# mchitten/keto

Measured on AMD Instinct MI355X. Metric: permission checks/sec (batched, whole node) + traversal HBM GB/s vs roofline, higher is better.
Workload: dtype u32 ids / u64 bitmasks (integer)

## Files before the change

include/ketogpu.h:

```cpp
#ifndef KETOGPU_H
#define KETOGPU_H

#include <stddef.h>
#include <stdint.h>

#ifdef __cplusplus
extern "C" {
#endif

#define KETOGPU_ABI_VERSION 9

#define KETOGPU_OK 0
#define KETOGPU_ENOTFOUND 1
#define KETOGPU_EINVAL 2
#define KETOGPU_EDEVICE 3
#define KETOGPU_ENOMEM 4
#define KETOGPU_ECOLLISION 5

#define KETOGPU_SUBJECT_ID 0
#define KETOGPU_SUBJECT_SET 1
#define KETOGPU_SUBJECT_NIL (-1)

#define KETOGPU_NODE_NONE 0xFFFFFFFFu
#define KETOGPU_NODE_NOT_OWNED 0xFFFFFFFEu
// ... 197 lines not shown
int ketogpu_host_alloc(size_t bytes, void **out);
void ketogpu_host_free(void *p);

typedef struct ketogpu_multi ketogpu_multi;
int ketogpu_multi_new(const ketogpu_snapshot *s, const int32_t *devices, size_t num_devices,
                      const ketogpu_engine_opts *opts, ketogpu_multi **out);
void ketogpu_multi_free(ketogpu_multi *m);
size_t ketogpu_multi_size(const ketogpu_multi *m);
ketogpu_engine *ketogpu_multi_engine(ketogpu_multi *m, size_t i);
int ketogpu_multi_check_ids(ketogpu_multi *m, const uint32_t *roots, const uint32_t *targets, size_t n,
                            uint64_t *allowed_bits, uint64_t *flagged_bits);
int ketogpu_multi_check_ids_packed24(ketogpu_multi *m, const void *packed, size_t n, uint64_t *allowed_bits,
                                     uint64_t *flagged_bits);
void ketogpu_multi_range(size_t n, size_t parts, size_t i, size_t *begin, size_t *end);

int ketogpu_queries_upload(ketogpu_engine *e, const uint32_t *roots, const uint32_t *targets,
                           size_t n, ketogpu_queries **out);
int ketogpu_queries_run(ketogpu_engine *e, ketogpu_queries *q);
int ketogpu_queries_download(ketogpu_engine *e, const ketogpu_queries *q, uint64_t *allowed_bits,
                             uint64_t *flagged_bits);
int ketogpu_queries_run_async(ketogpu_engine *e, ketogpu_queries *q, int *queued);
int ketogpu_engine_wait(ketogpu_engine *e);
int ketogpu_engine_piped_full_requests(ketogpu_engine *e, uint64_t *out);
void ketogpu_queries_free(ketogpu_queries *q);

typedef struct {
    uint64_t checks;
    uint64_t rounds;
    uint64_t levels;
    uint64_t frontier_entries;
    uint64_t interior_edges;
    uint64_t rev_edges;
    uint64_t touched;
    uint64_t bytes_push;
    uint64_t bytes_pull;
    uint64_t bytes_total;
    double ms_push;
    double ms_pull;
    double ms_total;
    uint64_t push_launches;
    uint64_t overflow_retries;
    uint64_t spilled_units;
    uint64_t unit_rows;
    uint64_t unit_edges;
    uint64_t unit_rev;
    uint64_t bytes_unit;
// ... 255 lines not shown
} ketogpu_tier_steps;
int ketogpu_tier_new_steps(const ketogpu_tier_steps *steps, ketogpu_comm *comm, const ketogpu_tier_opts *opts,
                           ketogpu_tier **out);

int ketogpu_expand(const ketogpu_snapshot *s, const ketogpu_subject *subject, int32_t rest_depth,
                   ketogpu_tree **out);

#define KETOGPU_NODE_UNION 0
#define KETOGPU_NODE_LEAF 1
typedef struct {
    int32_t type;
    uint32_t num_children;
    ketogpu_subject subject;
} ketogpu_tree_node;
int ketogpu_tree_nodes(const ketogpu_tree *t, const ketogpu_tree_node **nodes, size_t *n);
int ketogpu_tree_json(const ketogpu_tree *t, char **json);
void ketogpu_tree_free(ketogpu_tree *t);

const char *ketogpu_last_error(void);
int ketogpu_abi_version(void);
void ketogpu_free(void *p);
int ketogpu_device_count(void);
int ketogpu_probe_random_lines(int device, uint64_t table_bytes, uint64_t requests, int reps, double *ms_per_launch);

#ifdef __cplusplus
}
#endif
#endif
```

keto_amd/_lib.py:

```python
import ctypes as C
import os

HERE = os.path.dirname(os.path.abspath(__file__))
LIB_PATH = os.environ.get("KETOGPU_LIB") or os.path.join(HERE, "libketogpu.so")

OK, ENOTFOUND, EINVAL, EDEVICE, ENOMEM, ECOLLISION = 0, 1, 2, 3, 4, 5
SUBJECT_ID, SUBJECT_SET, SUBJECT_NIL = 0, 1, -1
NODE_NONE = 0xFFFFFFFF
NODE_NOT_OWNED = 0xFFFFFFFE
BUILD_SORT = 1
ORDER_NULLS_LAST = 2
ORDERS = {"sqlite": 0, "mysql-bin": 0, "cockroach": 0, "postgres": ORDER_NULLS_LAST}
BUILD_WRITABLE = 4
WRITE_REASONS = {0: "applied", 1: "not_writable", 2: "wildcard", 3: "poison", 4: "class", 5: "ambiguous",
                 6: "full", 7: "reserve", 8: "fanout"}
NODE_UNION, NODE_LEAF = 0, 1


class KetoError(Exception):

    NAMES = {ENOTFOUND: "not_found", EINVAL: "invalid", EDEVICE: "device", ENOMEM: "nomem", ECOLLISION: "collision"}

    def __init__(self, code, msg=""):
        super().__init__(f"{self.NAMES.get(code, code)}: {msg}")
# ... 286 lines not shown
    "ketogpu_snapshot_set_namespaces": (C.c_int, [vp, C.POINTER(Namespace), sz, C.POINTER(vp)]),
    "ketogpu_snapshot_write": (C.c_int, [vp, C.POINTER(RowBatch), C.POINTER(RowBatch), C.POINTER(WriteResult)]),
    "ketogpu_snapshot_version": (C.c_uint64, [vp]),
    "ketogpu_engine_sync": (C.c_int, [vp, C.POINTER(C.c_double), C.POINTER(C.c_uint64)]),
    "ketogpu_engine_check_graph": (C.c_int, [vp, C.POINTER(C.c_uint64)]),
    "ketogpu_resolve": (C.c_int, [vp, C.POINTER(CheckRequest), C.POINTER(u32), C.POINTER(u32)]),
    "ketogpu_resolve_batch": (C.c_int, [vp, C.POINTER(RequestBatch), vp, vp, vp]),
    "ketogpu_engine_new": (C.c_int, [vp, C.POINTER(EngineOpts), C.POINTER(vp)]),
    "ketogpu_engine_free": (None, [vp]),
    "ketogpu_engine_set_events": (C.c_int, [vp, C.c_int]),
    "ketogpu_check": (C.c_int, [vp, C.POINTER(CheckRequest), sz, vp, vp]),
    "ketogpu_check_ids": (C.c_int, [vp, vp, vp, sz, vp, vp]),
    "ketogpu_packed24_bytes": (sz, [sz]),
    "ketogpu_pack24": (C.c_int, [vp, vp, sz, vp]),
    "ketogpu_unpack24": (C.c_int, [vp, sz, vp, vp]),
    "ketogpu_snapshot_packed24_ok": (C.c_int, [vp]),
    "ketogpu_check_ids_packed24": (C.c_int, [vp, vp, sz, vp, vp]),
    "ketogpu_engine_last_request_path": (C.c_int, [vp, C.POINTER(i32)]),
    "ketogpu_queries_upload": (C.c_int, [vp, vp, vp, sz, C.POINTER(vp)]),
    "ketogpu_queries_run": (C.c_int, [vp, vp]),
    "ketogpu_queries_run_async": (C.c_int, [vp, vp, C.POINTER(C.c_int)]),
    "ketogpu_engine_wait": (C.c_int, [vp]),
    "ketogpu_engine_piped_full_requests": (C.c_int, [vp, C.POINTER(C.c_uint64)]),
    "ketogpu_probe_random_lines": (C.c_int, [C.c_int, C.c_uint64, C.c_uint64, C.c_int, C.POINTER(C.c_double)]),
    "ketogpu_queries_download": (C.c_int, [vp, vp, vp, vp]),
    "ketogpu_queries_free": (None, [vp]),
    "ketogpu_engine_last_stats": (C.c_int, [vp, C.POINTER(RunStats)]),
    "ketogpu_expand": (C.c_int, [vp, C.POINTER(Subject), i32, C.POINTER(vp)]),
    "ketogpu_tree_nodes": (C.c_int, [vp, C.POINTER(C.POINTER(TreeNode)), C.POINTER(sz)]),
    "ketogpu_tree_json": (C.c_int, [vp, C.POINTER(vp)]),
    "ketogpu_tree_free": (None, [vp]),
    "ketogpu_last_error": (C.c_char_p, []),
    "ketogpu_abi_version": (C.c_int, []),
    "ketogpu_free": (None, [vp]),
    "ketogpu_device_count": (C.c_int, []),
    "ketogpu_host_alloc": (C.c_int, [sz, C.POINTER(vp)]),
    "ketogpu_host_free": (None, [vp]),
    "ketogpu_multi_new": (C.c_int, [vp, vp, sz, C.POINTER(EngineOpts), C.POINTER(vp)]),
    "ketogpu_multi_free": (None, [vp]),
    "ketogpu_multi_size": (sz, [vp]),
    "ketogpu_multi_engine": (vp, [vp, sz]),
    "ketogpu_multi_check_ids": (C.c_int, [vp, vp, vp, sz, vp, vp]),
    "ketogpu_multi_check_ids_packed24": (C.c_int, [vp, vp, sz, vp, vp]),
    "ketogpu_multi_range": (None, [sz, sz, sz, C.POINTER(sz), C.POINTER(sz)]),
    "ketogpu_shard_builder_new": (C.c_int, [C.POINTER(Namespace), sz, C.POINTER(ShardOpts), C.POINTER(vp)]),
    "ketogpu_shard_builder_append": (C.c_int, [vp, C.POINTER(RowBatch)]),
    "ketogpu_shard_builder_finish": (C.c_int, [vp, C.POINTER(vp)]),
# ... 80 lines not shown
```

keto_amd/build.py:

```python
import os
import subprocess
import sys

HERE = os.path.dirname(os.path.abspath(__file__))
ROOT = os.path.dirname(HERE)
CSRC = os.path.join(HERE, "csrc")
LIB = os.path.join(HERE, "libketogpu.so")
SYNTH_LIB = os.path.join(HERE, "libketosynth.so")
HIPCC = os.environ.get("HIPCC", "/opt/rocm/bin/hipcc")
ARCH = os.environ.get("KETOGPU_ARCH", "gfx950")

SOURCES = ["snapshot.cpp", "snapshot_write.cpp", "snapshot_io.cpp", "host_engine.cpp", "multi_engine.cpp", "shard.cpp", "device_engine.hip", "partition.hip", "comm.cpp", "part_round.cpp", "tier.cpp", "core_index.cpp", "labels.cpp", "probe.hip", "packed24.cpp"]
HEADERS = ["ketogpu_internal.hpp", "device_util.hpp", "part_round.hpp", "tier.hpp", "core_index.hpp", "labels.hpp", os.path.join("..", "..", "include", "ketogpu.h")]


def kernel_source_hash():
    import hashlib
    h = hashlib.sha256()
    for f in ("device_engine.hip", "device_util.hpp", "core_index.hpp", "core_index.cpp", "labels.hpp", "labels.cpp"):
        with open(os.path.join(CSRC, f), "rb") as fh:
            h.update(fh.read())
    return h.hexdigest()[:16]


def _stale(out, deps):
    deps = list(deps) + [os.path.abspath(__file__)]
    if not os.path.exists(out):
        return True
    t = os.path.getmtime(out)
    return any(os.path.getmtime(d) > t for d in deps)


def _run(cmd):
    print("+", " ".join(cmd), flush=True)
    subprocess.run(cmd, check=True)


def build(force=False, jobs=4):
    objdir = os.path.join(HERE, "build")
    os.makedirs(objdir, exist_ok=True)
    hdrs = [os.path.join(CSRC, h) for h in HEADERS]
    objs = []
# ... 59 lines not shown
```

keto_amd/csrc/device_engine.hip:

```cpp
#include <hip/hip_runtime.h>

#include <algorithm>
#include <atomic>
#include <chrono>
#include <cstring>
#include <functional>
#include <map>
#include <mutex>
#include <string>
#include <thread>
#include <type_traits>
#include <vector>

#include "core_index.hpp"
#include "device_util.hpp"
#include "labels.hpp"
#include "tier.hpp"
#include "ketogpu_internal.hpp"

using namespace ketogpu;
using namespace kdev;

namespace {

constexpr int kBlock = 256;
constexpr int kItems = 4;
constexpr int kTile = kBlock * kItems;
constexpr uint32_t kDynBase = 0x80000000u;

struct DevGraph {
    const uint64_t *fint_off;
    const uint32_t *fint_col;
    const uint64_t *rev_off;
    const uint32_t *rev_col;
    const uint32_t *row_amb;
    uint32_t Ni, Nx, N;
    uint32_t both_max, seed_max;
    uint64_t seed_shift;
// ... 2111 lines not shown
            }
        }
    }
    const uint64_t units = (n + SH::U - 1) / SH::U;
#pragma unroll 1
    for (int k = 0; k < K; k++) {
        const uint64_t unit = (uint64_t)blockIdx.x * K + k;
        if (unit >= units) break;
        uint32_t rk = r[0], tk = t[0];
#pragma unroll
        for (int j = 1; j < K; j++)
            if (j == k) rk = r[j], tk = t[j];
        lite_unit<SH, CL>(S, g, frec, brec, CL ? core_load_rows(g, frec, brec, rk, tk) : bidi_load_rows(g, rk, tk),
                          allowed, unit, spill_out, spill_count, stats);
        __syncthreads();
    }
}

struct LabelGraph {
    const uint32_t *P, *S;
    uint32_t ni;
};
constexpr int kRestShards = 64, kRestStride = 32;
struct LabelRest {
    uint32_t *list;
    unsigned int *count, *next_count;
    uint64_t cap;
    uint4 *rec = nullptr;
};
template <int HS, int HP>
struct alignas(16) LabelShared {
    uint32_t S[16 * (HS + 4)], P[16 * (HP + 4)];
};

__device__ __forceinline__ bool label_find_n(const uint32_t *S, uint32_t n, uint32_t x) {
    const uint32_t n0 = n;
    uint32_t lo = 0;
    while (n) {
        const uint32_t half = n >> 1;
        if (S[lo + half] < x) {
            lo += half + 1;
            n -= half + 1;
        } else {
            n = half;
        }
    }
// ... 52 lines not shown
    const uint4 u = *reinterpret_cast<const uint4 *>(L + 8 * blk);
    const bool lo = min(min(u.x ^ x, u.y ^ x), min(u.z ^ x, u.w ^ x)) == 0;
    if constexpr (NB == 1) {
        return lo;
    } else {
        const uint4 v = *reinterpret_cast<const uint4 *>(L + 8 * blk + 4);
        const bool hi = min(min(v.x ^ x, v.y ^ x), min(v.z ^ x, v.w ^ x)) == 0;
        return lo | (hi & (blk != (uint32_t)(NB - 1)));
    }
}

template <int E, int H>
__device__ __forceinline__ bool label_lookup(const uint32_t *row, uint32_t x) {
    return label_block8<E>(row + kHeadFixed, x);
}

#ifndef KETO_LABEL_MEET
#define KETO_LABEL_MEET 0
#endif

template <int HS, int HP, bool TAIL = false>
__device__ __forceinline__ void label_unit(LabelShared<HS, HP> &sh, const LabelGraph &L, uint32_t r_lane,
                                           uint32_t t_lane, uint64_t *allowed, const uint64_t unit,
                                           const LabelRest &R, const LabelRest &F, unsigned long long *stats) {
    static_assert((HS == 8 || HS == 16 || HS == 32 || HS == 64) && (HP == 8 || HP == 16 || HP == 32 || HP == 64),
                  "heads of 8, 16, 32 or 64 words");
    constexpr int SW = HS / 4, PW = HP / 4;
    constexpr uint32_t CS = HS - kHeadFixed, CP = HP - kHeadFixed;
    const uint32_t lane = threadIdx.x & 63, q = lane >> 2, sub = lane & 3;
    const uint32_t r = (uint32_t)__shfl((int)r_lane, (int)q, 64), t = (uint32_t)__shfl((int)t_lane, (int)q, 64);
    const bool some = r != KETOGPU_NODE_NONE && t != KETOGPU_NODE_NONE;
    const bool valid = some && r < kDynBase;
    uint32_t sw[SW], pw[PW];
#pragma unroll
    for (int k = 0; k < SW; k++) sw[k] = 0xFFFFFFFFu;
#pragma unroll
    for (int k = 0; k < PW; k++) pw[k] = 0xFFFFFFFFu;
    if (valid) {
        label_head_load<SW>(L.S + (uint64_t)t * HS, sub, sw);
        label_head_load<PW>(L.P + (uint64_t)r * HP, sub, pw);
    }
    const uint32_t ns = label_word<SW, 0>(sw), np = label_word<PW, 0>(pw);
    const bool labelled = valid && ns != kNoLabel && np != kNoLabel;
    const uint64_t smask = (uint64_t)label_word<SW, 2>(sw) | (uint64_t)label_word<SW, 3>(sw) << 32;
    const uint64_t pmask = (uint64_t)label_word<PW, 2>(pw) | (uint64_t)label_word<PW, 3>(pw) << 32;
    uint32_t *Sl = sh.S + q * (HS + 4), *Pl = sh.P + q * (HP + 4);
    label_to_lds<SW>(Sl, sw, sub);
    label_to_lds<PW>(Pl, pw, sub);
    const uint32_t *Se = Sl + kHeadFixed, *Pe = Pl + kHeadFixed;
    const uint32_t shard = (uint32_t)(unit % kRestShards);
    {
        const bool rest = sub == 0 && some && !labelled;
        const uint32_t at = lds_append(rest, R.count + shard * kRestStride);
        if (rest) R.list[shard * R.cap + at] = (uint32_t)(unit * 16 + q);
    }
    wave_sync();
    bool hit = labelled && (smask & pmask) != 0;
    const bool s_body = sub * SW >= kHeadFixed;
    uint32_t es = 0;
#pragma unroll
    for (int k = 0; k < SW; k++) es += (k >= (int)kHeadFixed || s_body) && sw[k] < L.ni;
    es += (uint32_t)__builtin_amdgcn_update_dpp(0, (int)es, 0xB1, 0xf, 0xf, false);
    es += (uint32_t)__builtin_amdgcn_update_dpp(0, (int)es, 0x4E, 0xf, 0xf, false);
    if (!labelled) es = 0;
    const uint32_t ep = min(np, CP);
    {
        bool head = false, body = false;
#pragma unroll
        for (int k = 0; k < SW; k++) (k < (int)kHeadFixed ? head : body) |= sw[k] == r;
        hit |= labelled && r >= L.ni && (body | (head & s_body));
    }
    if (labelled && !hit) {
        if (KETO_LABEL_MEET == 2) {
// ... 87 lines not shown
    x = (x | x >> 3) & 0x0303030303030303ull;
    x = (x | x >> 6) & 0x000F000F000F000Full;
    x = (x | x >> 12) & 0x000000FF000000FFull;
    x = (x | x >> 24) & 0xFFFFull;
    if (lane == 0) {
        reinterpret_cast<uint16_t *>(allowed)[unit] = (uint16_t)x;
        if (stats) {
            atomicAdd(&stat_slot(stats)[0], (unsigned long long)rows);
            atomicAdd(&stat_slot(stats)[2], (unsigned long long)ent);
        }
    }
}

__device__ __forceinline__ void label_clear_next(const LabelRest &R, const LabelRest &F) {
    if (blockIdx.x == 0 && threadIdx.x < 64) {
        R.next_count[threadIdx.x * kRestStride] = 0u;
        F.next_count[threadIdx.x * kRestStride] = 0u;
    }
}

template <int HS, int HP>
__global__ __launch_bounds__(64) void label_kernel(LabelGraph L, const uint32_t *roots, const uint32_t *targets,
                                                   uint64_t n, uint64_t *allowed, LabelRest R, LabelRest F,
                                                   unsigned long long *stats, uint64_t unit0) {
    __shared__ LabelShared<HS, HP> sh;
    if (unit0 == 0) label_clear_next(R, F);
    const uint64_t units = (n + 15) / 16;
    const uint64_t unit = unit0 + blockIdx.x;
    uint32_t r, t;
    bidi_load_rt<16>(unit, units, roots, targets, n, r, t);
    label_unit<HS, HP>(sh, L, r, t, allowed, unit, R, F, stats);
    if (unit + 1 == units && threadIdx.x == 0)
        for (uint64_t u = units; u < (units + 3) / 4 * 4; u++) reinterpret_cast<uint16_t *>(allowed)[u] = 0;
}

template <int HS, int HP>
__global__ __launch_bounds__(256) void label_host_kernel(DevGraph g, LabelGraph L, const uint32_t *hr,
                                                         const uint32_t *ht, uint32_t *dr, uint32_t *dt, uint64_t n,
                                                         uint64_t *allowed, LabelRest R, LabelRest F,
                                                         unsigned long long *stats, unsigned long long *first_bad) {
    __shared__ LabelShared<HS, HP> sh[4];
    __shared__ uint32_t rq[2][64];
    const uint32_t wave = threadIdx.x >> 6, lane = threadIdx.x & 63;
    label_clear_next(R, F);
    if (wave == 0) {
        uint32_t r[4], t[4];
        host_unit_requests<4>(g, hr, ht, dr, dt, n, first_bad, r, t);
        if (lane < 16)
#pragma unroll
            for (int k = 0; k < 4; k++) rq[0][16 * k + lane] = r[k], rq[1][16 * k + lane] = t[k];
    }
    __syncthreads();
    const uint64_t units = (n + 15) / 16;
    const uint64_t unit = (uint64_t)blockIdx.x * 4 + wave;
    if (unit >= units) return;
    const uint32_t rk = lane < 16 ? rq[0][16 * wave + lane] : KETOGPU_NODE_NONE;
    const uint32_t tk = lane < 16 ? rq[1][16 * wave + lane] : KETOGPU_NODE_NONE;
    label_unit<HS, HP>(sh[wave], L, rk, tk, allowed, unit, R, F, stats);
}

__device__ __forceinline__ void packed24_decode(uint32_t *raw, const uint64_t *src, uint64_t w0, uint64_t nwords,
                                                uint32_t lane, uint32_t &r, uint32_t &t) {
    if (lane < 48) {
        const uint64_t w = w0 + lane < nwords ? src[w0 + lane] : 0ull;
        *reinterpret_cast<uint2 *>(raw + 2 * lane) = make_uint2((uint32_t)w, (uint32_t)(w >> 32));
    }
    wave_sync();
    const uint32_t k = (3 * lane) >> 1;
    const uint64_t v = ((uint64_t)raw[k + 1] << 32 | raw[k]) >> ((lane & 1) * 16);
    r = (uint32_t)v & 0xFFFFFFu;
    t = (uint32_t)(v >> 24) & 0xFFFFFFu;
    if (r == 0xFFFFFFu) r = KETOGPU_NODE_NONE;
    if (t == 0xFFFFFFu) t = KETOGPU_NODE_NONE;
}

template <int HS, int HP>
__global__ __launch_bounds__(256) void label_host_packed_kernel(DevGraph g, LabelGraph L, const uint64_t *hp,
                                                                uint32_t *dr, uint32_t *dt, uint64_t n,
                                                                uint64_t *allowed, LabelRest R, LabelRest F,
                                                                unsigned long long *stats,
                                                                unsigned long long *first_bad) {
// ... 5 lines not shown
        uint32_t r, t;
        packed24_decode(&rq[0][0], hp, (uint64_t)blockIdx.x * 48, (6 * n + 7) / 8, lane, r, t);
        const uint64_t c = (uint64_t)blockIdx.x * 64 + lane;
        if (c < n) {
            if ((r != KETOGPU_NODE_NONE && r >= g.Nx) || (t != KETOGPU_NODE_NONE && t >= g.N)) {
                atomicMin(first_bad, (unsigned long long)c);
                r = t = KETOGPU_NODE_NONE;
            }
            dr[c] = r;
            dt[c] = t;
        } else {
            r = t = KETOGPU_NODE_NONE;
        }
        wave_sync();
        rq[0][lane] = r;
        rq[1][lane] = t;
    }
    __syncthreads();
    const uint64_t units = (n + 15) / 16;
    const uint64_t unit = (uint64_t)blockIdx.x * 4 + wave;
    if (unit >= units) return;
    const uint32_t rk = lane < 16 ? rq[0][16 * wave + lane] : KETOGPU_NODE_NONE;
    const uint32_t tk = lane < 16 ? rq[1][16 * wave + lane] : KETOGPU_NODE_NONE;
    label_unit<HS, HP>(sh[wave], L, rk, tk, allowed, unit, R, F, stats);
}

__host__ __device__ constexpr uint32_t full_stage(int HS, int HP) { return HS >= 64 || HP >= 64 ? 256u : 128u; }

template <int HS, int HP, uint32_t kStage, int kPre, int kFly>
__device__ __forceinline__ uint64_t label_dense_units(uint32_t *stage, const LabelGraph &L, uint64_t *allowed,
                                                      const LabelRest &F, const uint32_t c, const uint32_t first_u,
                                                      const uint32_t stride) {
    static_assert(kStage % 4 == 0, "16-byte aligned rows");
    const uint32_t lane = threadIdx.x, q = lane >> 2, sub = lane & 3;
    const uint32_t nu = (c + 15) / 16;
    const uint32_t incl = wave_incl_sum_u32(nu);
    const uint64_t units = (uint64_t)__builtin_amdgcn_readlane((int)incl, 63);
    uint32_t *row = stage + q * kStage;
    uint64_t ent = 0;
    for (uint64_t u = first_u; u < units; u += stride) {
        const uint32_t shard = (uint32_t)__builtin_ctzll(__ballot(incl > u));
        const uint32_t first = (uint32_t)__builtin_amdgcn_readlane((int)(incl - nu), (int)shard);
        const uint32_t cs = (uint32_t)__builtin_amdgcn_readlane((int)c, (int)shard);
        const uint64_t j = (u - first) * 16 + (lane & 15);
        uint4 r0 = make_uint4(KETOGPU_NODE_NONE, 0, 0, 0), r1 = make_uint4(0, 0, 0, 0);
        if (lane < 16 && j < cs) {
            const uint4 *rec = F.rec + 2 * (shard * F.cap + j);
// ... 59 lines not shown
template <int HS, int HP>
__global__ __launch_bounds__(64) void label_full_kernel(LabelGraph L, uint64_t *allowed, LabelRest R, LabelRest F,
                                                        unsigned int *total_rest, unsigned int *total_full,
                                                        unsigned long long *stats, unsigned long long *mirror) {
    constexpr uint32_t kFullStage = full_stage(HS, HP);
    __shared__ alignas(16) uint32_t stage[16 * kFullStage];
    const uint32_t lane = threadIdx.x;
    const uint32_t c = F.count[lane * kRestStride];
    if (blockIdx.x == 0) {
        const uint32_t tr = wave_sum_all(R.count[lane * kRestStride]), tf = wave_sum_all(c);
        if (lane == 0) *total_rest = tr, *total_full = tf;
        if (mirror && lane < 12)
            mirror[lane] = lane == 8 ? (unsigned long long)tr : lane == 11 ? (unsigned long long)tf << 32 : 0ull;
    }
    const uint64_t ent =
        label_dense_units<HS, HP, kFullStage, 16, (int)kFullStage / 16>(stage, L, allowed, F, c, blockIdx.x, gridDim.x);
    const uint32_t e = wave_sum_all((uint32_t)ent);
    if (stats && lane == 0 && e) atomicAdd(&stat_slot(stats)[2], (unsigned long long)e);
}

template <int HS, int HP, bool TAIL>
__global__ __launch_bounds__(64) void label_carry_kernel(LabelGraph L, const uint32_t *roots, const uint32_t *targets,
                                                         uint64_t n, uint64_t *allowed, LabelRest R, LabelRest F,
                                                         LabelRest Fd, uint64_t *allowed_d, uint32_t D) {
    __shared__ LabelShared<HS, HP> sh;
    static_assert(sizeof(LabelShared<HS, HP>) == 64 * (HS + HP + 8), "the dense role's stage");
    if (blockIdx.x < D) {
        label_dense_units<HS, HP, HS + HP + 8, 4, 2>(reinterpret_cast<uint32_t *>(&sh), L, allowed_d, Fd,
                                                     Fd.count[threadIdx.x * kRestStride], blockIdx.x, D);
        return;
    }
    if (blockIdx.x == D) {
        R.next_count[threadIdx.x * kRestStride] = 0u;
        F.next_count[threadIdx.x * kRestStride] = 0u;
    }
    const uint64_t units = (n + 15) / 16;
    const uint64_t unit = blockIdx.x - D;
    uint32_t r, t;
    bidi_load_rt<16>(unit, units, roots, targets, n, r, t);
    label_unit<HS, HP, TAIL>(sh, L, r, t, allowed, unit, R, F, nullptr);
    if (unit + 1 == units && threadIdx.x == 0)
        for (uint64_t u = units; u < (units + 3) / 4 * 4; u++) reinterpret_cast<uint16_t *>(allowed)[u] = 0;
}

template <class SH>
__global__ __launch_bounds__(64) void label_rest_kernel(DevGraph g, const FRec *frec, const FRec *brec,
                                                        const uint32_t *roots, const uint32_t *targets,
                                                        uint64_t *allowed, LabelRest R, unsigned int *total,
                                                        uint32_t *out, unsigned int *out_count,
                                                        unsigned long long *stats) {
    __shared__ SH S;
    const uint32_t lane = threadIdx.x;
    const uint32_t c = R.count[lane * kRestStride];
    const uint32_t nu = (c + 15) / 16;
    const uint32_t incl = wave_incl_sum_u32(nu);
    const uint64_t units = (uint64_t)__builtin_amdgcn_readlane((int)incl, 63);
    const uint32_t listed = wave_sum_all(c);
    if (blockIdx.x == 0 && lane == 0) *total = listed;
    for (uint64_t u = blockIdx.x; u < units; u += gridDim.x) {
        const uint32_t shard = (uint32_t)__builtin_ctzll(__ballot(incl > u));
        const uint32_t first = (uint32_t)__builtin_amdgcn_readlane((int)(incl - nu), (int)shard);
        const uint32_t cs = (uint32_t)__builtin_amdgcn_readlane((int)c, (int)shard);
        const uint64_t j = (u - first) * 16 + lane;
// ... 1407 lines not shown
    uint64_t *h_ctr = nullptr;
    unsigned long long *d_hctr = nullptr;
    std::vector<void *> owned;
    ketogpu_run_stats last{};
    std::vector<hipEvent_t> ev_pool;
    size_t ev_used = 0;
    bool use_units = true;
    int wave_u = 8;
    bool use_v2 = true;
    bool use_bidi = true;
    bool use_lite = false;
    bool use_core = false;
    const FRec *core_rec[2] = {nullptr, nullptr};
    uint64_t core_blk[2] = {0, 0};
    uint32_t core_blk_log[2] = {0, 0}, core_block[2] = {0, 0};
    uint64_t core_overflow[2] = {0, 0};
    uint32_t closure_cap[2] = {64, 64};
    bool use_label = false;
    LabelGraph lgraph{};
    static constexpr unsigned kPipe = 2;
    static constexpr unsigned kLabelSets = 3 * kPipe;
    unsigned int *rest_counts = nullptr;
    uint64_t label_calls = 0;
    LabelRest label_rest(uint64_t n) {
        const uint64_t units = (n + 15) / 16;
        const unsigned set = (unsigned)(label_calls % kLabelSets), next = (unsigned)((label_calls + kPipe) % kLabelSets);
        return LabelRest{spill_units, rest_counts + set * kRestShards * kRestStride,
                         rest_counts + next * kRestShards * kRestStride, 16 * ((units + kRestShards - 1) / kRestShards)};
    }
    LabelRest label_full(uint64_t n) {
        const uint64_t units = (n + 15) / 16;
        const unsigned set = (unsigned)(label_calls % kLabelSets), next = (unsigned)((label_calls + kPipe) % kLabelSets);
        return LabelRest{nullptr, rest_counts + (kLabelSets + set) * kRestShards * kRestStride,
                         rest_counts + (kLabelSets + next) * kRestShards * kRestStride,
                         16 * ((units + kRestShards - 1) / kRestShards), full_rec + (uint64_t)set * 2 * spill_cap};
    }
    uint4 *full_rec = nullptr;
    bool fuse_reduce = [] {
        const char *e = getenv("KETOGPU_LABEL_FUSE");
        return !e || atoi(e) != 0;
    }();
    bool label_clean = false;
    bool lean_call = false;
    bool pipelined_req = false, queued = false;
    hipStream_t pipe_s[kPipe] = {};
    bool pipe_used[kPipe] = {};
    const ketogpu_queries *pipe_q[kPipe] = {};
    bool label_defer = [] {
        const char *e = getenv("KETOGPU_LABEL_DEFER");
        return !e || atoi(e) != 0;
    }();
    int done_mode = [] {
        const char *e = getenv("KETOGPU_LABEL_DONE_EVENT");
        return !e ? 2 : !strcmp(e, "record") ? 0 : !strcmp(e, "nofence") ? 1 : 2;
    }();
    struct PendingDense {
        bool on = false;
        ketogpu_queries *q = nullptr;
// ... 124 lines not shown
        bool units = true;
        int u = 16;
        int wpe = 1;
        int lite = 0;
    };
    std::vector<Candidate> candidates;
    struct BidiCfg {
        int hlog, bt, f, lf;
        int u = 16;
        int wpe = 1;
        int lite = 0;
        bool operator==(const BidiCfg &o) const {
            return hlog == o.hlog && bt == o.bt && f == o.f && lf == o.lf && u == o.u && wpe == o.wpe &&
                   lite == o.lite;
        }
    };
    BidiCfg bidi_cfg{9, 64, KETO_F1, 7};

    void launch_bidi(const BidiCfg &c, unsigned grid, unsigned pad, const Batch &q, const uint32_t *parents,
                     const unsigned int *in_count, uint32_t *out, unsigned int *out_count, unsigned long long *stats,
                     unsigned long long *stp, uint64_t unit0 = 0, hipStream_t stream = nullptr, bool chunked = false) {
        if (!stream) stream = this->stream;
        if (c.lite == 3) {
            label_dispatch([&](auto hs, auto hp) {
                KLAUNCH((label_kernel<decltype(hs)::value, decltype(hp)::value>), dim3(grid), dim3(64), pad, stream,
                        lgraph, q.roots, q.targets, q.n, q.allowed, label_rest(q.n), label_full(q.n), stats, unit0);
            });
            return;
        }
        if (c.lite == 2) {
#define KETO_CORE_K(SH)                                                                                       \
    KLAUNCH((lite_kernel<SH, true>), dim3(grid), dim3(64), pad, stream, gcore(), core_rec[0], core_rec[1], q.roots, \
            q.targets, q.n, q.allowed, out, out_count, stats, unit0, stp)
            if (core_shape == 1)
                KETO_CORE_K(CoreShapeS);
            else if (core_shape == 2)
                KETO_CORE_K(CoreShapeM);
            else
                KETO_CORE_K(LiteShape);
#undef KETO_CORE_K
            return;
        }
        if (c.lite) {
            if (c.u == 32)
                KLAUNCH((lite_kernel<LiteShape32>), dim3(grid), dim3(64), pad, stream, g, frec, brec, q.roots,
                        q.targets, q.n, q.allowed, out, out_count, stats, unit0, stp);
            else
                KLAUNCH((lite_kernel<LiteShape>), dim3(grid), dim3(64), pad, stream, g, frec, brec, q.roots, q.targets,
                        q.n, q.allowed, out, out_count, stats, unit0, stp);
// ... 1047 lines not shown
        g.hub_words = hub_words;
        n_hubs = H;
        hub_build_ms = std::chrono::duration<double, std::milli>(std::chrono::steady_clock::now() - t0).count();
        if (cascade_log)
            fprintf(stderr, "[hubs] %u hubs (interior rows >= %llu entries: smallest hub row %llu) built in %.1f ms\n",
                    H, (unsigned long long)kHubDeg,
                    (unsigned long long)(s.fint_off[hub_nodes.back() + 1] - s.fint_off[hub_nodes.back()]), hub_build_ms);
        std::vector<uint32_t>().swap(hub_of_h);
        if (trials_left && use_units) candidates.push_back({false, 0, 0, 0, 0, 0, false});
    }
    const uint32_t *up_hub(const std::vector<uint32_t> &v) {
        uint32_t *p = dupload(v);
        owned.push_back(p);
        return p;
    }

    void ensure_spill(uint64_t n) {
        if (n <= spill_cap) return;
        flush_dense_all();
        if (pipe_busy() || pipe_q[0]) HIP_CHECK(hipDeviceSynchronize());
        for (void *p : {(void *)spill_units, (void *)spill_roots, (void *)spill_targets, (void *)spill_allowed,
                        (void *)spill_flags})
            if (p) (void)hipFree(p);
        spill_cap = std::max<uint64_t>(n + 2048, 1024);
        spill_units = dalloc<uint32_t>(2 * spill_cap);
        if (full_rec) (void)hipFree(full_rec);
        full_rec = dalloc<uint4>(kLabelSets * 2 * spill_cap);
        spill_roots = dalloc<uint32_t>(spill_cap);
        spill_targets = dalloc<uint32_t>(spill_cap);
        spill_allowed = dalloc<uint64_t>(spill_cap / 64 + 1);
        spill_flags = dalloc<uint64_t>(spill_cap / 64 + 1);
    }

    unsigned long long *stat_out() { return st.stats + 8 + 8 * kStatSlots; }

    void read_unit_stats(uint64_t out[3]) {
        KLAUNCH(stats_reduce_kernel, dim3(1), dim3(kBlock), 0, stream, st.stats + 8, 2, stat_out(), nullptr, 0,
                EmitReq{});
        HIP_CHECK(hipMemcpyAsync(h_ctr + 32, stat_out(), 6 * sizeof(uint64_t), hipMemcpyDeviceToHost, stream));
        HIP_CHECK(hipStreamSynchronize(stream));
        for (int k = 0; k < 3; k++) out[k] = h_ctr[32 + k] + h_ctr[35 + k];
    }

    uint32_t read_spill_count() {
        HIP_CHECK(hipMemcpyAsync(h_ctr + 12, spill_count, sizeof(unsigned int), hipMemcpyDeviceToHost, stream));
        HIP_CHECK(hipStreamSynchronize(stream));
        return (uint32_t)h_ctr[12];
// ... 164 lines not shown
            HIP_CHECK(hipEventRecord(b, stream));
            unit_ev.push_back({a, b});
            left = read_spill_count();
            rs.spilled_units += left;
            rs.push_launches++;
            if (left)
                HIP_CHECK(hipMemcpyAsync(list[0], list[1], left * sizeof(uint32_t), hipMemcpyDeviceToDevice, stream));
            return left;
        }
        uint64_t units = (q.n + 15) / 16;
        uint64_t left = 0;
        if (use_v2 || (use_lite && use_bidi)) {
            if (use_bidi) {
                const bool direct = src && src->mapped && pipe_direct &&
                                    (bidi_cfg == BidiCfg{9, 64, KETO_F1, 7, 16, 1} || bidi_cfg.lite);
                const bool light = light_begin && (direct || !src);
                hipEvent_t a = light ? light_begin : ev(), b = light ? nullptr : ev();
                if (!light) HIP_CHECK(hipEventRecord(a, stream));
                const uint64_t bunits = (q.n + bidi_cfg.u - 1) / bidi_cfg.u;
                if (!src && carry_call) {
                    PendingDense p = pend[cur_pipe];
                    pend[cur_pipe] = PendingDense{};
                    const unsigned D = p.on ? piped_grid() : 0u;
                    label_dispatch([&](auto hs, auto hp) {
                        if (label_tail)
                            KLAUNCH((label_carry_kernel<decltype(hs)::value, decltype(hp)::value, true>),
                                    dim3(D + (unsigned)bunits), dim3(64), lds_pad, stream, lgraph, q.roots, q.targets,
                                    q.n, q.allowed, label_rest(q.n), label_full(q.n), p.F, p.allowed, D);
                        else
                            KLAUNCH((label_carry_kernel<decltype(hs)::value, decltype(hp)::value, false>),
                                    dim3(D + (unsigned)bunits), dim3(64), lds_pad, stream, lgraph, q.roots, q.targets,
                                    q.n, q.allowed, label_rest(q.n), label_full(q.n), p.F, p.allowed, D);
                    });
                    if (p.q) p.q->pass = 2;
                } else if (!src) {
                    launch_bidi(bidi_cfg, (unsigned)bunits, lds_pad, q, nullptr, nullptr, list[0], &spill_count[0],
                                lean_call ? nullptr : st.stats, stamps);
                } else if (direct) {
#define KETO_HOST_K(K)                                                                                     \
    do {                                                                                                   \
        if (bidi_cfg.lite == 3)                                                                            \
            launch_label_host(q, src, bunits);                                                             \
        else if (bidi_cfg.lite == 2 && core_shape == 1)                                                    \
            KLAUNCH((lite_host_kernel<K, CoreShapeS, true>), dim3((unsigned)((bunits + K - 1) / K)), dim3(64), \
                    0, stream, gcore(), core_rec[0], core_rec[1], src->roots, src->targets, io->d_roots,   \
                    io->d_targets, q.n, q.allowed, list[0], &spill_count[0], st.stats, d_bad);              \
        else if (bidi_cfg.lite == 2 && core_shape == 2)                                                    \
            KLAUNCH((lite_host_kernel<K, CoreShapeM, true>), dim3((unsigned)((bunits + K - 1) / K)), dim3(64), \
                    0, stream, gcore(), core_rec[0], core_rec[1], src->roots, src->targets, io->d_roots,   \
                    io->d_targets, q.n, q.allowed, list[0], &spill_count[0], st.stats, d_bad);              \
        else if (bidi_cfg.lite == 2)                                                                       \
            KLAUNCH((lite_host_kernel<K, LiteShape, true>), dim3((unsigned)((bunits + K - 1) / K)), dim3(64), \
                    0, stream, gcore(), core_rec[0], core_rec[1], src->roots, src->targets, io->d_roots,   \
                    io->d_targets, q.n, q.allowed, list[0], &spill_count[0], st.stats, d_bad);              \
        else if (bidi_cfg.lite && bidi_cfg.u == 32)                                                        \
// ... 728 lines not shown
    e->pipelined_req = false;
    if (queued) *queued = e->queued ? 1 : 0;
    API_END
}

int ketogpu_engine_wait(ketogpu_engine *e) {
    API_BEGIN
    if (!e) throw Error(KETOGPU_EINVAL, "null argument");
    std::lock_guard<std::mutex> lk(e->mu);
    HIP_CHECK(hipSetDevice(e->device));
    e->drain_pipe();
    HIP_CHECK(hipStreamSynchronize(e->stream));
    API_END
}

int ketogpu_engine_piped_full_requests(ketogpu_engine *e, uint64_t *out) {
    API_BEGIN
    if (!e || !out) throw Error(KETOGPU_EINVAL, "null argument");
    std::lock_guard<std::mutex> lk(e->mu);
    *out = e->piped_full_known ? e->piped_full : 0;
    API_END
}

int ketogpu_queries_download(ketogpu_engine *e, const ketogpu_queries *q, uint64_t *allowed_bits,
                             uint64_t *flagged_bits) {
    API_BEGIN
    if (!e || !q) throw Error(KETOGPU_EINVAL, "null argument");
    std::lock_guard<std::mutex> lk(e->mu);
    e->download(const_cast<ketogpu_queries &>(*q), allowed_bits, flagged_bits);
    API_END
}

void ketogpu_queries_free(ketogpu_queries *q) {
    if (q && q->pass == 1 && q->eng) {
        ketogpu_engine *e = q->eng;
        std::lock_guard<std::mutex> lk(e->mu);
        try {
            HIP_CHECK(hipSetDevice(e->device));
            for (unsigned k = 0; k < ketogpu_engine::kPipe; k++)
                if (e->pend[k].on && e->pend[k].q == q) e->flush_dense(k);
        } catch (const Error &) {
            for (unsigned k = 0; k < ketogpu_engine::kPipe; k++)
                if (e->pend[k].q == q) e->pend[k] = ketogpu_engine::PendingDense{};
        }
    }
    delete q;
// ... 226 lines not shown
```

keto_amd/csrc/probe.hip:

```cpp
#include <hip/hip_runtime.h>

#include <cstdint>

#include "../../include/ketogpu.h"

namespace {

__global__ __launch_bounds__(64) void probe_lines_kernel(const uint32_t *table, uint64_t lines, const uint32_t *rq,
                                                         uint64_t n, uint16_t *out) {
    const uint32_t lane = threadIdx.x, q = lane >> 2, sub = lane & 3;
    const uint64_t i0 = (uint64_t)blockIdx.x * 16;
    uint32_t a = 0, b = 0;
    if (lane < 16 && i0 + lane < n) a = rq[2 * (i0 + lane)], b = rq[2 * (i0 + lane) + 1];
    a = (uint32_t)__shfl((int)a, (int)q, 64);
    b = (uint32_t)__shfl((int)b, (int)q, 64);
    uint32_t v = 0;
    if (i0 + q < n) {
        const uint4 *x = reinterpret_cast<const uint4 *>(table + (a % lines) * 32) + 2 * sub;
        const uint4 *y = reinterpret_cast<const uint4 *>(table + (b % lines) * 32) + 2 * sub;
        const uint4 x0 = x[0], x1 = x[1], y0 = y[0], y1 = y[1];
        v = x0.x ^ x0.y ^ x0.z ^ x0.w ^ x1.x ^ x1.y ^ x1.z ^ x1.w ^ y0.x ^ y0.y ^ y0.z ^ y0.w ^ y1.x ^ y1.y ^ y1.z ^ y1.w;
    }
    const uint64_t bits = __ballot((v & 0xF) == 3);
    if (lane == 0) out[blockIdx.x] = (uint16_t)(bits ^ (bits >> 16) ^ (bits >> 32) ^ (bits >> 48));
}

}

extern "C" int ketogpu_probe_random_lines(int device, uint64_t table_bytes, uint64_t requests, int reps,
                                          double *ms_per_launch) {
    if (!ms_per_launch || requests == 0 || reps <= 0 || table_bytes < (1u << 20)) return KETOGPU_EINVAL;
    *ms_per_launch = 0;
    if (hipSetDevice(device) != hipSuccess) return KETOGPU_EDEVICE;
    const uint64_t lines = table_bytes / 128;
    uint32_t *table = nullptr, *rq = nullptr;
    uint16_t *out = nullptr;
    hipStream_t s = nullptr;
    hipEvent_t e0 = nullptr, e1 = nullptr;
    int rc = KETOGPU_OK;
    auto ok = [&](hipError_t e) {
        if (e != hipSuccess && rc == KETOGPU_OK) rc = e == hipErrorOutOfMemory ? KETOGPU_ENOMEM : KETOGPU_EDEVICE;
        return rc == KETOGPU_OK;
    };
    const uint64_t grid = (requests + 15) / 16;
    if (ok(hipMalloc(&table, lines * 128)) && ok(hipMalloc(&rq, 8 * requests)) && ok(hipMalloc(&out, 2 * grid)) &&
        ok(hipStreamCreateWithFlags(&s, hipStreamNonBlocking)) && ok(hipEventCreate(&e0)) && ok(hipEventCreate(&e1)) &&
        ok(hipMemsetAsync(table, 0x5a, lines * 128, s))) {
        uint32_t *h = nullptr;
        if (ok(hipHostMalloc(&h, 8 * requests, hipHostMallocDefault))) {
// ... 30 lines not shown
```

Before: 24.78 billion.

## Remap label kernel workgroups so contiguous units land on the same XCD

Adds an XCD-aware block-to-unit permutation for the label and label-carry kernels. Round-robin dispatch across the 8 XCDs otherwise spreads neighbouring units over different L2 caches, so consecutive blocks are remapped to give each XCD contiguous chunks of 16 units. The grid is padded to a multiple of 8×chunk with early exit for the padding blocks, and rest-shard capacity and spill buffers grow to cover it. It is on by default via an env flag and includes a probe to check the hardware XCD mapping. The padding adds some empty workgroups, and chunked launches fall back to the plain order when they are misaligned.

```diff
diff --git a/include/ketogpu.h b/include/ketogpu.h
--- a/include/ketogpu.h
+++ b/include/ketogpu.h
@@ -243,6 +243,9 @@
 int ketogpu_queries_run_async(ketogpu_engine *e, ketogpu_queries *q, int *queued);
 int ketogpu_engine_wait(ketogpu_engine *e);
 int ketogpu_engine_piped_full_requests(ketogpu_engine *e, uint64_t *out);
+uint32_t ketogpu_label_xcd_chunk(void);
+uint64_t ketogpu_label_xcd_unit(uint32_t chunk, uint64_t u);
+uint64_t ketogpu_label_xcd_padded(uint32_t chunk, uint64_t units);
 void ketogpu_queries_free(ketogpu_queries *q);
 
 typedef struct {
@@ -544,6 +547,7 @@
 void ketogpu_free(void *p);
 int ketogpu_device_count(void);
 int ketogpu_probe_random_lines(int device, uint64_t table_bytes, uint64_t requests, int reps, double *ms_per_launch);
+int ketogpu_probe_xcd_map(int device, uint32_t blocks, uint32_t skip, uint32_t *out0, uint32_t *out1);
 
 #ifdef __cplusplus
 }
diff --git a/keto_amd/_lib.py b/keto_amd/_lib.py
--- a/keto_amd/_lib.py
+++ b/keto_amd/_lib.py
@@ -332,7 +332,11 @@
     "ketogpu_queries_run_async": (C.c_int, [vp, vp, C.POINTER(C.c_int)]),
     "ketogpu_engine_wait": (C.c_int, [vp]),
     "ketogpu_engine_piped_full_requests": (C.c_int, [vp, C.POINTER(C.c_uint64)]),
+    "ketogpu_label_xcd_chunk": (C.c_uint32, []),
+    "ketogpu_label_xcd_unit": (C.c_uint64, [C.c_uint32, C.c_uint64]),
+    "ketogpu_label_xcd_padded": (C.c_uint64, [C.c_uint32, C.c_uint64]),
     "ketogpu_probe_random_lines": (C.c_int, [C.c_int, C.c_uint64, C.c_uint64, C.c_int, C.POINTER(C.c_double)]),
+    "ketogpu_probe_xcd_map": (C.c_int, [C.c_int, C.c_uint32, C.c_uint32, vp, vp]),
     "ketogpu_queries_download": (C.c_int, [vp, vp, vp, vp]),
     "ketogpu_queries_free": (None, [vp]),
     "ketogpu_engine_last_stats": (C.c_int, [vp, C.POINTER(RunStats)]),
diff --git a/keto_amd/build.py b/keto_amd/build.py
--- a/keto_amd/build.py
+++ b/keto_amd/build.py
@@ -11,13 +11,13 @@
 ARCH = os.environ.get("KETOGPU_ARCH", "gfx950")
 
 SOURCES = ["snapshot.cpp", "snapshot_write.cpp", "snapshot_io.cpp", "host_engine.cpp", "multi_engine.cpp", "shard.cpp", "device_engine.hip", "partition.hip", "comm.cpp", "part_round.cpp", "tier.cpp", "core_index.cpp", "labels.cpp", "probe.hip", "packed24.cpp"]
-HEADERS = ["ketogpu_internal.hpp", "device_util.hpp", "part_round.hpp", "tier.hpp", "core_index.hpp", "labels.hpp", os.path.join("..", "..", "include", "ketogpu.h")]
+HEADERS = ["ketogpu_internal.hpp", "device_util.hpp", "part_round.hpp", "tier.hpp", "core_index.hpp", "labels.hpp", "label_xcd.hpp", os.path.join("..", "..", "include", "ketogpu.h")]
 
 
 def kernel_source_hash():
     import hashlib
     h = hashlib.sha256()
-    for f in ("device_engine.hip", "device_util.hpp", "core_index.hpp", "core_index.cpp", "labels.hpp", "labels.cpp"):
+    for f in ("device_engine.hip", "device_util.hpp", "core_index.hpp", "core_index.cpp", "labels.hpp", "labels.cpp", "label_xcd.hpp"):
         with open(os.path.join(CSRC, f), "rb") as fh:
             h.update(fh.read())
     return h.hexdigest()[:16]
diff --git a/keto_amd/csrc/device_engine.hip b/keto_amd/csrc/device_engine.hip
--- a/keto_amd/csrc/device_engine.hip
+++ b/keto_amd/csrc/device_engine.hip
@@ -14,6 +14,7 @@
 
 #include "core_index.hpp"
 #include "device_util.hpp"
+#include "label_xcd.hpp"
 #include "labels.hpp"
 #include "tier.hpp"
 #include "ketogpu_internal.hpp"
@@ -2171,6 +2172,8 @@
     uint32_t ni;
 };
 constexpr int kRestShards = 64, kRestStride = 32;
+constexpr uint32_t kLabelXcdChunk = KETO_LABEL_XCD_CHUNK;
+static_assert(kLabelXcdChunk >= 1 && (kLabelXcdChunk & (kLabelXcdChunk - 1)) == 0, "KETO_LABEL_XCD_CHUNK: a power of two");
 struct LabelRest {
     uint32_t *list;
     unsigned int *count, *next_count;
@@ -2269,7 +2272,8 @@
 template <int HS, int HP, bool TAIL = false>
 __device__ __forceinline__ void label_unit(LabelShared<HS, HP> &sh, const LabelGraph &L, uint32_t r_lane,
                                            uint32_t t_lane, uint64_t *allowed, const uint64_t unit,
-                                           const LabelRest &R, const LabelRest &F, unsigned long long *stats) {
+                                           const LabelRest &R, const LabelRest &F, unsigned long long *stats,
+                                           const uint64_t shard_of) {
     static_assert((HS == 8 || HS == 16 || HS == 32 || HS == 64) && (HP == 8 || HP == 16 || HP == 32 || HP == 64),
                   "heads of 8, 16, 32 or 64 words");
     constexpr int SW = HS / 4, PW = HP / 4;
@@ -2295,7 +2299,7 @@
     label_to_lds<SW>(Sl, sw, sub);
     label_to_lds<PW>(Pl, pw, sub);
     const uint32_t *Se = Sl + kHeadFixed, *Pe = Pl + kHeadFixed;
-    const uint32_t shard = (uint32_t)(unit % kRestShards);
+    const uint32_t shard = (uint32_t)(shard_of % kRestShards);
     {
         const bool rest = sub == 0 && some && !labelled;
         const uint32_t at = lds_append(rest, R.count + shard * kRestStride);
@@ -2429,14 +2433,17 @@
 template <int HS, int HP>
 __global__ __launch_bounds__(64) void label_kernel(LabelGraph L, const uint32_t *roots, const uint32_t *targets,
                                                    uint64_t n, uint64_t *allowed, LabelRest R, LabelRest F,
-                                                   unsigned long long *stats, uint64_t unit0) {
+                                                   unsigned long long *stats, uint64_t unit0, uint32_t m,
+                                                   uint32_t xcd) {
     __shared__ LabelShared<HS, HP> sh;
     if (unit0 == 0) label_clear_next(R, F);
     const uint64_t units = (n + 15) / 16;
-    const uint64_t unit = unit0 + blockIdx.x;
+    const uint64_t local = xcd ? label_xcd_unit<kLabelXcdChunk>(blockIdx.x) : blockIdx.x;
+    if (local >= m) return;
+    const uint64_t unit = unit0 + local;
     uint32_t r, t;
     bidi_load_rt<16>(unit, units, roots, targets, n, r, t);
-    label_unit<HS, HP>(sh, L, r, t, allowed, unit, R, F, stats);
+    label_unit<HS, HP>(sh, L, r, t, allowed, unit, R, F, stats, unit0 + blockIdx.x);
     if (unit + 1 == units && threadIdx.x == 0)
         for (uint64_t u = units; u < (units + 3) / 4 * 4; u++) reinterpret_cast<uint16_t *>(allowed)[u] = 0;
 }
@@ -2463,7 +2470,7 @@
     if (unit >= units) return;
     const uint32_t rk = lane < 16 ? rq[0][16 * wave + lane] : KETOGPU_NODE_NONE;
     const uint32_t tk = lane < 16 ? rq[1][16 * wave + lane] : KETOGPU_NODE_NONE;
-    label_unit<HS, HP>(sh[wave], L, rk, tk, allowed, unit, R, F, stats);
+    label_unit<HS, HP>(sh[wave], L, rk, tk, allowed, unit, R, F, stats, unit);
 }
 
 __device__ __forceinline__ void packed24_decode(uint32_t *raw, const uint64_t *src, uint64_t w0, uint64_t nwords,
@@ -2515,7 +2522,7 @@
     if (unit >= units) return;
     const uint32_t rk = lane < 16 ? rq[0][16 * wave + lane] : KETOGPU_NODE_NONE;
     const uint32_t tk = lane < 16 ? rq[1][16 * wave + lane] : KETOGPU_NODE_NONE;
-    label_unit<HS, HP>(sh[wave], L, rk, tk, allowed, unit, R, F, stats);
+    label_unit<HS, HP>(sh[wave], L, rk, tk, allowed, unit, R, F, stats, unit);
 }
 
 __host__ __device__ constexpr uint32_t full_stage(int HS, int HP) { return HS >= 64 || HP >= 64 ? 256u : 128u; }
@@ -2621,7 +2628,8 @@
 template <int HS, int HP, bool TAIL>
 __global__ __launch_bounds__(64) void label_carry_kernel(LabelGraph L, const uint32_t *roots, const uint32_t *targets,
                                                          uint64_t n, uint64_t *allowed, LabelRest R, LabelRest F,
-                                                         LabelRest Fd, uint64_t *allowed_d, uint32_t D) {
+                                                         LabelRest Fd, uint64_t *allowed_d, uint32_t D,
+                                                         uint32_t xcd) {
     __shared__ LabelShared<HS, HP> sh;
     static_assert(sizeof(LabelShared<HS, HP>) == 64 * (HS + HP + 8), "the dense role's stage");
     if (blockIdx.x < D) {
@@ -2634,10 +2642,12 @@
         F.next_count[threadIdx.x * kRestStride] = 0u;
     }
     const uint64_t units = (n + 15) / 16;
-    const uint64_t unit = blockIdx.x - D;
+    const uint64_t u = blockIdx.x - D;
+    const uint64_t unit = xcd ? label_xcd_unit<kLabelXcdChunk>(u) : u;
+    if (unit >= units) return;
     uint32_t r, t;
     bidi_load_rt<16>(unit, units, roots, targets, n, r, t);
-    label_unit<HS, HP, TAIL>(sh, L, r, t, allowed, unit, R, F, nullptr);
+    label_unit<HS, HP, TAIL>(sh, L, r, t, allowed, unit, R, F, nullptr, u);
     if (unit + 1 == units && threadIdx.x == 0)
         for (uint64_t u = units; u < (units + 3) / 4 * 4; u++) reinterpret_cast<uint16_t *>(allowed)[u] = 0;
 }
@@ -4091,18 +4101,25 @@
     static constexpr unsigned kLabelSets = 3 * kPipe;
     unsigned int *rest_counts = nullptr;
     uint64_t label_calls = 0;
+    static uint64_t label_cap(uint64_t units) {
+        return 16 * ((label_xcd_padded<kLabelXcdChunk>(units) + kRestShards - 1) / kRestShards);
+    }
+    bool label_xcd = [] {
+        const char *e = getenv("KETOGPU_LABEL_XCD");
+        return !e || atoi(e) != 0;
+    }();
     LabelRest label_rest(uint64_t n) {
         const uint64_t units = (n + 15) / 16;
         const unsigned set = (unsigned)(label_calls % kLabelSets), next = (unsigned)((label_calls + kPipe) % kLabelSets);
         return LabelRest{spill_units, rest_counts + set * kRestShards * kRestStride,
-                         rest_counts + next * kRestShards * kRestStride, 16 * ((units + kRestShards - 1) / kRestShards)};
+                         rest_counts + next * kRestShards * kRestStride, label_cap(units)};
     }
     LabelRest label_full(uint64_t n) {
         const uint64_t units = (n + 15) / 16;
         const unsigned set = (unsigned)(label_calls % kLabelSets), next = (unsigned)((label_calls + kPipe) % kLabelSets);
         return LabelRest{nullptr, rest_counts + (kLabelSets + set) * kRestShards * kRestStride,
                          rest_counts + (kLabelSets + next) * kRestShards * kRestStride,
-                         16 * ((units + kRestShards - 1) / kRestShards), full_rec + (uint64_t)set * 2 * spill_cap};
+                         label_cap(units), full_rec + (uint64_t)set * 2 * spill_cap};
     }
     uint4 *full_rec = nullptr;
     bool fuse_reduce = [] {
@@ -4273,9 +4290,14 @@
                      unsigned long long *stp, uint64_t unit0 = 0, hipStream_t stream = nullptr, bool chunked = false) {
         if (!stream) stream = this->stream;
         if (c.lite == 3) {
+            constexpr uint64_t group = kXcdClasses * kLabelXcdChunk;
+            const bool xcd = label_xcd && (!chunked || (unit0 % group == 0 &&
+                                                        (grid % group == 0 || unit0 + grid == (q.n + 15) / 16)));
+            const unsigned wgs = xcd ? (unsigned)label_xcd_padded<kLabelXcdChunk>(grid) : grid;
             label_dispatch([&](auto hs, auto hp) {
-                KLAUNCH((label_kernel<decltype(hs)::value, decltype(hp)::value>), dim3(grid), dim3(64), pad, stream,
-                        lgraph, q.roots, q.targets, q.n, q.allowed, label_rest(q.n), label_full(q.n), stats, unit0);
+                KLAUNCH((label_kernel<decltype(hs)::value, decltype(hp)::value>), dim3(wgs), dim3(64), pad, stream,
+                        lgraph, q.roots, q.targets, q.n, q.allowed, label_rest(q.n), label_full(q.n), stats, unit0,
+                        (uint32_t)grid, xcd ? 1u : 0u);
             });
             return;
         }
@@ -5369,7 +5391,7 @@
         for (void *p : {(void *)spill_units, (void *)spill_roots, (void *)spill_targets, (void *)spill_allowed,
                         (void *)spill_flags})
             if (p) (void)hipFree(p);
-        spill_cap = std::max<uint64_t>(n + 2048, 1024);
+        spill_cap = std::max<uint64_t>(n + 2048 + 16 * kXcdClasses * kLabelXcdChunk, 1024);
         spill_units = dalloc<uint32_t>(2 * spill_cap);
         if (full_rec) (void)hipFree(full_rec);
         full_rec = dalloc<uint4>(kLabelSets * 2 * spill_cap);
@@ -5580,15 +5602,17 @@
                     PendingDense p = pend[cur_pipe];
                     pend[cur_pipe] = PendingDense{};
                     const unsigned D = p.on ? piped_grid() : 0u;
+                    const unsigned wgs = label_xcd ? (unsigned)label_xcd_padded<kLabelXcdChunk>(bunits) : (unsigned)bunits;
+                    const uint32_t xcd = label_xcd ? 1u : 0u;
                     label_dispatch([&](auto hs, auto hp) {
                         if (label_tail)
                             KLAUNCH((label_carry_kernel<decltype(hs)::value, decltype(hp)::value, true>),
-                                    dim3(D + (unsigned)bunits), dim3(64), lds_pad, stream, lgraph, q.roots, q.targets,
-                                    q.n, q.allowed, label_rest(q.n), label_full(q.n), p.F, p.allowed, D);
+                                    dim3(D + wgs), dim3(64), lds_pad, stream, lgraph, q.roots, q.targets,
+                                    q.n, q.allowed, label_rest(q.n), label_full(q.n), p.F, p.allowed, D, xcd);
                         else
                             KLAUNCH((label_carry_kernel<decltype(hs)::value, decltype(hp)::value, false>),
-                                    dim3(D + (unsigned)bunits), dim3(64), lds_pad, stream, lgraph, q.roots, q.targets,
-                                    q.n, q.allowed, label_rest(q.n), label_full(q.n), p.F, p.allowed, D);
+                                    dim3(D + wgs), dim3(64), lds_pad, stream, lgraph, q.roots, q.targets,
+                                    q.n, q.allowed, label_rest(q.n), label_full(q.n), p.F, p.allowed, D, xcd);
                     });
                     if (p.q) p.q->pass = 2;
                 } else if (!src) {
@@ -6363,6 +6387,28 @@
     API_END
 }
 
+uint32_t ketogpu_label_xcd_chunk(void) { return kLabelXcdChunk; }
+
+uint64_t ketogpu_label_xcd_unit(uint32_t chunk, uint64_t u) {
+    if (chunk == kLabelXcdChunk) return label_xcd_unit<kLabelXcdChunk>(u);
+    switch (chunk) {
+    case 2: return label_xcd_unit<2>(u);
+    case 16: return label_xcd_unit<16>(u);
+    case 64: return label_xcd_unit<64>(u);
+    default: return UINT64_MAX;
+    }
+}
+
+uint64_t ketogpu_label_xcd_padded(uint32_t chunk, uint64_t units) {
+    if (chunk == kLabelXcdChunk) return label_xcd_padded<kLabelXcdChunk>(units);
+    switch (chunk) {
+    case 2: return label_xcd_padded<2>(units);
+    case 16: return label_xcd_padded<16>(units);
+    case 64: return label_xcd_padded<64>(units);
+    default: return UINT64_MAX;
+    }
+}
+
 int ketogpu_queries_download(ketogpu_engine *e, const ketogpu_queries *q, uint64_t *allowed_bits,
                              uint64_t *flagged_bits) {
     API_BEGIN
diff --git a/keto_amd/csrc/label_xcd.hpp b/keto_amd/csrc/label_xcd.hpp
--- /dev/null
+++ b/keto_amd/csrc/label_xcd.hpp
@@ -0,0 +1,28 @@
+#pragma once
+#include <cstdint>
+
+#if defined(__HIPCC__)
+#define KETO_XCD_HD __host__ __device__
+#else
+#define KETO_XCD_HD
+#endif
+
+#ifndef KETO_LABEL_XCD_CHUNK
+#define KETO_LABEL_XCD_CHUNK 16
+#endif
+
+constexpr uint32_t kXcdClasses = 8;
+
+template <uint32_t C>
+KETO_XCD_HD inline uint64_t label_xcd_unit(uint64_t u) {
+    static_assert(C >= 1, "chunk");
+    constexpr uint64_t group = (uint64_t)kXcdClasses * C;
+    const uint64_t j = u % group;
+    return u - j + (j % kXcdClasses) * C + j / kXcdClasses;
+}
+
+template <uint32_t C>
+KETO_XCD_HD constexpr uint64_t label_xcd_padded(uint64_t units) {
+    constexpr uint64_t group = (uint64_t)kXcdClasses * C;
+    return (units + group - 1) / group * group;
+}
diff --git a/keto_amd/csrc/probe.hip b/keto_amd/csrc/probe.hip
--- a/keto_amd/csrc/probe.hip
+++ b/keto_amd/csrc/probe.hip
@@ -25,6 +25,41 @@
     if (lane == 0) out[blockIdx.x] = (uint16_t)(bits ^ (bits >> 16) ^ (bits >> 32) ^ (bits >> 48));
 }
 
+__global__ __launch_bounds__(64) void probe_xcd_kernel(uint32_t *out, uint32_t skip) {
+    uint32_t xcc;
+    asm volatile("s_getreg_b32 %0, hwreg(HW_REG_XCC_ID, 0, 4)" : "=s"(xcc));
+    for (int k = 0; k < 64; k++) __builtin_amdgcn_s_sleep(32);
+    if (blockIdx.x >= skip && threadIdx.x == 0) out[blockIdx.x - skip] = xcc;
+}
+
+}
+
+extern "C" int ketogpu_probe_xcd_map(int device, uint32_t blocks, uint32_t skip, uint32_t *out0, uint32_t *out1) {
+    if (!out0 || !out1 || !blocks || (uint64_t)blocks + skip > (1u << 24)) return KETOGPU_EINVAL;
+    if (hipSetDevice(device) != hipSuccess) return KETOGPU_EDEVICE;
+    uint32_t *d[2] = {nullptr, nullptr};
+    hipStream_t s[2] = {nullptr, nullptr};
+    int rc = KETOGPU_OK;
+    auto ok = [&](hipError_t e) {
+        if (e != hipSuccess && rc == KETOGPU_OK) rc = e == hipErrorOutOfMemory ? KETOGPU_ENOMEM : KETOGPU_EDEVICE;
+        return rc == KETOGPU_OK;
+    };
+    for (int k = 0; k < 2; k++)
+        if (ok(hipMalloc(&d[k], 4ull * blocks)) && ok(hipStreamCreateWithFlags(&s[k], hipStreamNonBlocking)))
+            ok(hipMemsetAsync(d[k], 0xFF, 4ull * blocks, s[k]));
+    if (rc == KETOGPU_OK && ok(hipStreamSynchronize(s[0])) && ok(hipStreamSynchronize(s[1]))) {
+        for (int k = 0; k < 2; k++) probe_xcd_kernel<<<dim3(skip + blocks), dim3(64), 0, s[k]>>>(d[k], skip);
+        ok(hipGetLastError());
+        uint32_t *out[2] = {out0, out1};
+        for (int k = 0; k < 2; k++)
+            if (ok(hipStreamSynchronize(s[k]))) ok(hipMemcpy(out[k], d[k], 4ull * blocks, hipMemcpyDeviceToHost));
+    }
+    for (int k = 0; k < 2; k++) {
+        if (s[k]) (void)hipStreamSynchronize(s[k]);
+        if (s[k]) (void)hipStreamDestroy(s[k]);
+        if (d[k]) (void)hipFree(d[k]);
+    }
+    return rc;
 }
 
 extern "C" int ketogpu_probe_random_lines(int device, uint64_t table_bytes, uint64_t requests, int reps,
```

New measurement: 24.61 billion. About the same (-0.7%).
